# pothosware/PothosComms

Measured on NVIDIA B200. Metric: FIR Msamples/s (cf32, 256 taps) at 1/2/4/8 B200; % HBM roofline; vs host CPU, higher is better.
Workload: dtype f32

## Files before the change

### pothoscomms_b200/csrc/fir_os.cu

```cuda
#include <algorithm>
#include <cmath>
#include <complex>
#include <cstdlib>
#include <vector>

#include "bulk.cuh"
#include "fft.hpp"
#include "os64_core.cuh"

namespace b200c {

struct FirOs64Args {
    const void *in;
    void *out;
    const void *hf;
    const void *twa;
    const void *twb;
    const void *twf;
    long long n_in;
    long long n_out;
    long long in_stride, out_stride;
    int nchan;
    int K;
    int parts;
};

template <bool CONJ, bool SLOT_REV>
__device__ __forceinline__ void step_twiddle(c2 (&v)[64], const c2 *__restrict__ twa, const c2 *__restrict__ twb, const int t)
{
    c2 A[8], B[8];
#pragma unroll
    for (int i = 1; i < 8; i++) { A[i] = twa[i * 64 + t]; B[i] = twb[i * 64 + t]; }
#pragma unroll
    for (int a = 0; a < 8; a++)
#pragma unroll
        for (int b = 0; b < 8; b++) {
            const int j = 8 * a + b, r = SLOT_REV ? rev64(j) : j;
            if (a) v[r] = cmul_p<CONJ>(v[r], A[a]);
            if (b) v[r] = cmul_p<CONJ>(v[r], B[b]);
        }
}

constexpr int kBulkElems = 4098;

template <int MINB>
__global__ void __launch_bounds__(64, MINB) fir_os64_kernel(const FirOs64Args a)
{
    __shared__ __align__(16) c2 F[kOs64SmemElems];
    __shared__ __align__(8) unsigned long long bar;
    const int t = threadIdx.x;
    const c2 *__restrict__ twa = static_cast<const c2 *>(a.twa);
    const c2 *__restrict__ twb = static_cast<const c2 *>(a.twb);
    const int Km1 = a.K - 1;
    const int hop = 4096 - Km1;
    const long long nblk = (a.n_out + hop - 1) / hop;
    const long long tstep = gridDim.x, dch = tstep / nblk, dblk = tstep - dch * nblk;
    long long ch = (long long)blockIdx.x / nblk, blk = (long long)blockIdx.x - ch * nblk;
    auto bulk_src = [&](long long ch, long long blk, const c2 *&src) {
        if (ch >= a.nchan) return false;
        const long long base = blk * hop;
        const c2 *in = static_cast<const c2 *>(a.in) + ch * a.in_stride;
        const int mis = (int)(((reinterpret_cast<unsigned long long>(in) >> 3) + base) & 1);
        src = in + (base - mis);
        return base - mis >= 0 && base - mis + kBulkElems <= a.n_in;
    };
    if (t == 0) mbar_init(&bar, 1);
    __syncthreads();
    const c2 *src = nullptr;
    bool pending = bulk_src(ch, blk, src);
    if (pending && t == 0) bulk_load(F, src, kBulkElems * (unsigned)sizeof(c2), &bar);
    unsigned parity = 0;

    while (ch < a.nchan) {
        const long long base = blk * hop;
        long long nch = ch + dch, nblkpos = blk + dblk;
        if (nblkpos >= nblk) { nblkpos -= nblk; nch++; }
        const c2 *__restrict__ in = static_cast<const c2 *>(a.in) + ch * a.in_stride;
        const c2 *__restrict__ hf = static_cast<const c2 *>(a.hf) + ch * 4096;
        c2 *__restrict__ out = static_cast<c2 *>(a.out) + ch * a.out_stride;
        c2 v[64];
        if (pending) {
            const int mis = (int)(((reinterpret_cast<unsigned long long>(in) >> 3) + base) & 1);
            mbar_wait(&bar, parity);
            parity ^= 1;
#pragma unroll
            for (int n1 = 0; n1 < 64; n1++) v[rev64(n1)] = F[mis + 64 * n1 + t];
        } else {
#pragma unroll
            for (int n1 = 0; n1 < 64; n1++) {
                const long long g = base + 64 * n1 + t;
                v[rev64(n1)] = g < a.n_in ? __ldcg(in + g) : 0ull;
            }
        }
        dft64_dit<false>(v);
        step_twiddle<false, false>(v, twa, twb, t);
        __syncthreads();
#pragma unroll
        for (int k1 = 0; k1 < 64; k1++) F[k1 * kOs64Stride + t] = v[k1];
        __syncthreads();
#pragma unroll
        for (int n2 = 0; n2 < 64; n2++) v[rev64(n2)] = F[t * kOs64Stride + n2];
        dft64_dit<false>(v);
#pragma unroll
        for (int k2 = 0; k2 < 64; k2++) v[k2] = cmul_p<false>(v[k2], hf[64 * k2 + t]);
        dft64_dif<true>(v);
        step_twiddle<true, true>(v, twa, twb, t);
        __syncthreads();
#pragma unroll
        for (int n2 = 0; n2 < 64; n2++) F[t * kOs64Stride + n2] = v[rev64(n2)];
        __syncthreads();
#pragma unroll
        for (int k1 = 0; k1 < 64; k1++) v[k1] = F[k1 * kOs64Stride + t];
        __syncthreads();
        pending = bulk_src(nch, nblkpos, src);
        if (pending && t == 0) bulk_load(F, src, kBulkElems * (unsigned)sizeof(c2), &bar);
        dft64_dif<true>(v);
        c2 *o = out + (base - Km1);
        if (base + hop <= a.n_out) {
#pragma unroll
            for (int n1 = 0; n1 < 64; n1++) {
                const int i = 64 * n1 + t;
                if (i >= Km1) __stcg(o + i, v[rev64(n1)]);
            }
        } else {
#pragma unroll
            for (int n1 = 0; n1 < 64; n1++) {
                const int i = 64 * n1 + t;
                if (i >= Km1 && base + i - Km1 < a.n_out) __stcg(o + i, v[rev64(n1)]);
            }
        }
        ch = nch; blk = nblkpos;
    }
}

constexpr int kOs64Groups = 4;
__global__ void __launch_bounds__(64 * kOs64Groups, 1) fir_os64p_kernel(const FirOs64Args a)
{
    extern __shared__ __align__(16) c2 os64p_dyn[];
    __shared__ __align__(8) unsigned long long bars[kOs64Groups];
    const int g = threadIdx.x >> 6, t = threadIdx.x & 63;
    c2 *F = os64p_dyn + g * kOs64SmemElems;
    c2 *TW = os64p_dyn + kOs64Groups * kOs64SmemElems;
    c2 *HF = TW + 4096;
    unsigned long long *bar = &bars[g];
    auto gsync = [&] { asm volatile("bar.sync %0, 64;" ::"r"(g + 1) : "memory"); };
    const int Km1 = a.K - 1;
    const int hop = 4096 - Km1;
    const long long nblk = (a.n_out + hop - 1) / hop;
    const long long parts = a.parts, ntask = (long long)a.nchan * parts;
    const long long bstep = parts * kOs64Groups;
    auto bulk_src = [&](long long ch, long long blk, const c2 *&src) {
        if (ch >= a.nchan || blk >= nblk) return false;
        const long long base = blk * hop;
        const c2 *in = static_cast<const c2 *>(a.in) + ch * a.in_stride;
        const int mis = (int)(((reinterpret_cast<unsigned long long>(in) >> 3) + base) & 1);
        src = in + (base - mis);
        return base - mis >= 0 && base - mis + kBulkElems <= a.n_in;
    };
    long long task = blockIdx.x;
    if (t == 0) mbar_init(bar, 1);
    gsync();
    const c2 *src = nullptr;
    bool pending = task < ntask && bulk_src(task / parts, (task % parts) * kOs64Groups + g, src);
    if (pending && t == 0) bulk_load(F, src, kBulkElems * (unsigned)sizeof(c2), bar);
    unsigned parity = 0;
    {
        const c2 *__restrict__ twf = static_cast<const c2 *>(a.twf);
        for (int i = threadIdx.x; i < 4096; i += 64 * kOs64Groups) TW[i] = twf[i];
    }
    long long staged = -1;
    for (; task < ntask; task += gridDim.x) {
        const long long ch = task / parts, first = (task - ch * parts) * kOs64Groups + g;
        if (ch != staged) {
            const c2 *__restrict__ hfg = static_cast<const c2 *>(a.hf) + ch * 4096;
            for (int i = threadIdx.x; i < 4096; i += 64 * kOs64Groups) HF[i] = __ldg(hfg + i);
            staged = ch;
        }
        __syncthreads();
        const c2 *__restrict__ in = static_cast<const c2 *>(a.in) + ch * a.in_stride;
        c2 *__restrict__ out = static_cast<c2 *>(a.out) + ch * a.out_stride;
        for (long long blk = first; blk < nblk; blk += bstep) {
            const long long base = blk * hop;
            c2 v[64];
            if (pending) {
                const int mis = (int)(((reinterpret_cast<unsigned long long>(in) >> 3) + base) & 1);
                mbar_wait(bar, parity);
                parity ^= 1;
#pragma unroll
                for (int n1 = 0; n1 < 64; n1++) v[rev64(n1)] = F[mis + 64 * n1 + t];
            } else {
#pragma unroll
                for (int n1 = 0; n1 < 64; n1++) {
                    const long long gi = base + 64 * n1 + t;
                    v[rev64(n1)] = gi < a.n_in ? __ldcg(in + gi) : 0ull;
                }
            }
            dft64_dit<false>(v);
#pragma unroll
            for (int k1 = 1; k1 < 64; k1++) v[k1] = cmul_p<false>(v[k1], TW[k1 * 64 + t]);
            gsync();
#pragma unroll
            for (int k1 = 0; k1 < 64; k1++) F[k1 * kOs64Stride + t] = v[k1];
            gsync();
#pragma unroll
            for (int n2 = 0; n2 < 64; n2++) v[rev64(n2)] = F[t * kOs64Stride + n2];
            dft64_dit<false>(v);
#pragma unroll
            for (int k2 = 0; k2 < 64; k2++) v[k2] = cmul_p<false>(v[k2], HF[64 * k2 + t]);
            dft64_dif<true>(v);
#pragma unroll
            for (int n2 = 1; n2 < 64; n2++) v[rev64(n2)] = cmul_p<true>(v[rev64(n2)], TW[n2 * 64 + t]);
            gsync();
#pragma unroll
            for (int n2 = 0; n2 < 64; n2++) F[t * kOs64Stride + n2] = v[rev64(n2)];
            gsync();
#pragma unroll
            for (int k1 = 0; k1 < 64; k1++) v[k1] = F[k1 * kOs64Stride + t];
            gsync();
            {
                const bool last = blk + bstep >= nblk;
                const long long nt = task + gridDim.x;
                pending = last ? (nt < ntask && bulk_src(nt / parts, (nt % parts) * kOs64Groups + g, src)) : bulk_src(ch, blk + bstep, src);
                if (pending && t == 0) bulk_load(F, src, kBulkElems * (unsigned)sizeof(c2), bar);
            }
            dft64_dif<true>(v);
            c2 *o = out + (base - Km1);
            if (base + hop <= a.n_out) {
#pragma unroll
                for (int n1 = 0; n1 < 64; n1++) {
                    const int i = 64 * n1 + t;
                    if (i >= Km1) __stcg(o + i, v[rev64(n1)]);
                }
            } else {
#pragma unroll
                for (int n1 = 0; n1 < 64; n1++) {
                    const int i = 64 * n1 + t;
                    if (i >= Km1 && base + i - Km1 < a.n_out) __stcg(o + i, v[rev64(n1)]);
                }
            }
        }
        __syncthreads();
    }
}


constexpr bool kOs32PartialTwiddles = false;

template <bool CONJ, bool SLOT_REV>
__device__ __forceinline__ void twiddle32(c2 (&v)[32], const c2 *__restrict__ tw, const int t)
{
    c2 A[8], B[4];
#pragma unroll
    for (int a = 1; a < 8; a++) A[a] = tw[(4 * a) * 32 + t];
#pragma unroll
    for (int b = 1; b < 4; b++) B[b] = tw[b * 32 + t];
#pragma unroll
    for (int k = 1; k < 32; k++) {
        const int a = k >> 2, b = k & 3, r = SLOT_REV ? rev32(k) : k;
        if (a) v[r] = cmul_p<CONJ>(v[r], A[a]);
        if (b) v[r] = cmul_p<CONJ>(v[r], B[b]);
    }
}

struct FirOs32Args {
    const void *in;
    void *out;
    const void *hf;
    const void *tw;
    long long n_in, n_out;
    long long in_stride, out_stride;
    int nchan;
    int K;
    int spread;
    int pdl;
};

constexpr int kOs32Landing = 1032;
template <int WARPS, int MINB, bool TABS = false, bool PT = kOs32PartialTwiddles, bool EARLY = false>
__global__ void __launch_bounds__(32 * WARPS, MINB) fir_os32_kernel(const FirOs32Args a)
{
    extern __shared__ __align__(16) c2 os32_dyn[];
    __shared__ __align__(16) c2 Fs[TABS ? 1 : WARPS][TABS ? 1 : kOs32SmemElems];
    __shared__ __align__(8) unsigned long long bars[WARPS];
    const int t = threadIdx.x & 31, w = threadIdx.x >> 5;
    c2 *F = TABS ? os32_dyn + w * kOs32SmemElems : Fs[TABS ? 0 : w];
    unsigned long long *bar = &bars[w];
    const c2 *__restrict__ tw = static_cast<const c2 *>(a.tw);
    const c2 *__restrict__ hf_tab = nullptr;
    c2 *Lb = F;
    if constexpr (TABS && EARLY) Lb = os32_dyn + WARPS * kOs32SmemElems + 2048 + w * kOs32Landing;
    const int Km1 = a.K - 1;
    const int hop = 1024 - Km1;
    const long long nblk = (a.n_out + hop - 1) / hop;
    const long long tstep = (long long)gridDim.x * WARPS, dch = tstep / nblk, dblk = tstep - dch * nblk;
    const long long task0 = a.spread ? (long long)w * gridDim.x + blockIdx.x : (long long)blockIdx.x * WARPS + w;
    long long ch = task0 / nblk, blk = task0 - ch * nblk;
    constexpr int kBulk = 1026;
    auto bulk_src = [&](long long ch, long long blk, const c2 *&src) {
        if (ch >= a.nchan) return false;
        const long long base = blk * hop;
        const c2 *in = static_cast<const c2 *>(a.in) + ch * a.in_stride;
        const int mis = (int)(((reinterpret_cast<unsigned long long>(in) >> 3) + base) & 1);
        src = in + (base - mis);
        return base - mis >= 0 && base - mis + kBulk <= a.n_in;
    };
    if (t == 0) mbar_init(bar, 1);
    __syncwarp();
    const c2 *src = nullptr;
    bool pending = bulk_src(ch, blk, src);
    unsigned parity = 0;
    if constexpr (TABS) {
        asm volatile("griddepcontrol.launch_dependents;");
        c2 *tab = os32_dyn + WARPS * kOs32SmemElems;
        const c2 *__restrict__ hf0 = static_cast<const c2 *>(a.hf);
        if (a.pdl) {
            for (int i = threadIdx.x; i < 1024; i += 32 * WARPS) { tab[i] = hf0[i]; tab[1024 + i] = tw[i]; }
            asm volatile("griddepcontrol.wait;" ::: "memory");
            if (pending && t == 0) bulk_load(Lb, src, kBulk * (unsigned)sizeof(c2), bar);
        } else {
            if (pending && t == 0) bulk_load(Lb, src, kBulk * (unsigned)sizeof(c2), bar);
            for (int i = threadIdx.x; i < 1024; i += 32 * WARPS) { tab[i] = hf0[i]; tab[1024 + i] = tw[i]; }
        }
        __syncthreads();
        hf_tab = tab; tw = tab + 1024;
    } else {
        if (pending && t == 0) bulk_load(Lb, src, kBulk * (unsigned)sizeof(c2), bar);
    }
    while (ch < a.nchan) {
        const long long base = blk * hop;
        long long nch = ch + dch, nblkpos = blk + dblk;
        if (nblkpos >= nblk) { nblkpos -= nblk; nch++; }
        const c2 *__restrict__ in = static_cast<const c2 *>(a.in) + ch * a.in_stride;
        const c2 *__restrict__ hf = TABS ? hf_tab : static_cast<const c2 *>(a.hf) + ch * 1024;
        c2 *__restrict__ out = static_cast<c2 *>(a.out) + ch * a.out_stride;
        c2 v[32];
        if (pending) {
            const int mis = (int)(((reinterpret_cast<unsigned long long>(in) >> 3) + base) & 1);
            mbar_wait(bar, parity);
            parity ^= 1;
#pragma unroll
            for (int n1 = 0; n1 < 32; n1++) v[rev32(n1)] = Lb[mis + 32 * n1 + t];
        } else {
#pragma unroll
            for (int n1 = 0; n1 < 32; n1++) {
                const long long g = base + 32 * n1 + t;
                v[rev32(n1)] = g < a.n_in ? __ldcg(in + g) : 0ull;
            }
        }
        if constexpr (TABS && EARLY) {
            __syncwarp();
            pending = bulk_src(nch, nblkpos, src);
            if (pending && t == 0) bulk_load(Lb, src, kBulk * (unsigned)sizeof(c2), bar);
        }
        dft32_dit<false>(v);
        if constexpr (PT) twiddle32<false, false>(v, tw, t);
        else {
#pragma unroll
            for (int k1 = 1; k1 < 32; k1++) v[k1] = cmul_p<false>(v[k1], tw[k1 * 32 + t]);
        }
        __syncwarp();
#pragma unroll
        for (int k1 = 0; k1 < 32; k1++) F[k1 * kOs32Stride + t] = v[k1];
        __syncwarp();
#pragma unroll
        for (int n2 = 0; n2 < 32; n2++) v[rev32(n2)] = F[t * kOs32Stride + n2];
        dft32_dit<false>(v);
#pragma unroll
        for (int k2 = 0; k2 < 32; k2++) v[k2] = cmul_p<false>(v[k2], hf[32 * k2 + t]);
        dft32_dif<true>(v);
        if constexpr (PT) twiddle32<true, true>(v, tw, t);
        else {
#pragma unroll
            for (int n2 = 1; n2 < 32; n2++) v[rev32(n2)] = cmul_p<true>(v[rev32(n2)], tw[n2 * 32 + t]);
        }
        __syncwarp();
#pragma unroll
        for (int n2 = 0; n2 < 32; n2++) F[t * kOs32Stride + n2] = v[rev32(n2)];
        __syncwarp();
#pragma unroll
        for (int k1 = 0; k1 < 32; k1++) v[k1] = F[k1 * kOs32Stride + t];
        if constexpr (!(TABS && EARLY)) {
            __syncwarp();
            pending = bulk_src(nch, nblkpos, src);
            if (pending && t == 0) bulk_load(F, src, kBulk * (unsigned)sizeof(c2), bar);
        }
        dft32_dif<true>(v);
        c2 *o = out + (base - Km1);
        if (base + hop <= a.n_out) {
#pragma unroll
            for (int n1 = 0; n1 < 32; n1++) {
                const int i = 32 * n1 + t;
                if (i >= Km1) __stcg(o + i, v[rev32(n1)]);
            }
        } else {
#pragma unroll
            for (int n1 = 0; n1 < 32; n1++) {
                const int i = 32 * n1 + t;
                if (i >= Km1 && base + i - Km1 < a.n_out) __stcg(o + i, v[rev32(n1)]);
            }
        }
        ch = nch; blk = nblkpos;
    }
}

B200C_HD constexpr float cos48(int e)
{
    constexpr float t[48] = {
        1.0f, 0.9914448857307434f, 0.9659258127212524f, 0.9238795042037964f, 0.8660253882408142f, 0.7933533191680908f,
        0.7071067690849304f, 0.6087614297866821f, 0.5f, 0.3826834261417389f, 0.258819043636322f, 0.13052618503570557f, 0.0f,
        -0.13052618503570557f, -0.258819043636322f, -0.3826834261417389f, -0.5f, -0.6087614297866821f, -0.7071067690849304f,
        -0.7933533191680908f, -0.8660253882408142f, -0.9238795042037964f, -0.9659258127212524f, -0.9914448857307434f, -1.0f,
        -0.9914448857307434f, -0.9659258127212524f, -0.9238795042037964f, -0.8660253882408142f, -0.7933533191680908f,
        -0.7071067690849304f, -0.6087614297866821f, -0.5f, -0.3826834261417389f, -0.258819043636322f, -0.13052618503570557f, 0.0f,
        0.13052618503570557f, 0.258819043636322f, 0.3826834261417389f, 0.5f, 0.6087614297866821f, 0.7071067690849304f,
        0.7933533191680908f, 0.8660253882408142f, 0.9238795042037964f, 0.9659258127212524f, 0.9914448857307434f};
    return t[e % 48];
}
B200C_HD constexpr float sin48(int e) { return cos48(e + 36); }

B200C_HD constexpr int rev16(int k) { return 4 * (k & 3) + (k >> 2); }
template <bool INV> B200C_HD void dft16_dif(c2 (&x)[16])
{
#pragma unroll
    for (int k = 0; k < 4; k++) {
        dft4_p<INV>(x[k], x[k + 4], x[k + 8], x[k + 12]);
        x[k + 4] = mul_w64<INV>(x[k + 4], 4 * k);
        x[k + 8] = mul_w64<INV>(x[k + 8], 8 * k);
        x[k + 12] = mul_w64<INV>(x[k + 12], 12 * k);
    }
#pragma unroll
    for (int g = 0; g < 4; g++) dft4_p<INV>(x[4 * g], x[4 * g + 1], x[4 * g + 2], x[4 * g + 3]);
}

B200C_HD c2 cmul_acc(c2 f, c2 w, c2 acc)
{
    float fx, fy, wx, wy;
    upk(f, fx, fy); upk(w, wx, wy);
    return fma2(f, pk(wx, wx), fma2(pk(-fy, fx), pk(wy, wy), acc));
}

struct FirOsX32Args {
    const void *in;
    void *out;
    const void *hx;
    const void *tw;
    const void *tw3;
    long long n_in, n_out;
    long long p0;
    int m0;
    int pdl;
};
constexpr int kX32Rows = 48, kX32SmemElems = kX32Rows * kOs32Stride;

constexpr int kX32TabElems = 3072 + 1536 + 1024;
template <int WARPS, int MINB, bool PT = false, bool SPLIT = false>
__global__ void __launch_bounds__(32 * WARPS, MINB) fir_os32x_kernel(const FirOsX32Args a)
{
    extern __shared__ __align__(16) c2 x32_smem[];
    __shared__ __align__(8) unsigned long long bars[WARPS];
    const int t = threadIdx.x & 31, wp = threadIdx.x >> 5;
    const c2 *__restrict__ tw = static_cast<const c2 *>(a.tw);
    const c2 *__restrict__ tw3 = static_cast<const c2 *>(a.tw3);
    const c2 *__restrict__ hx = static_cast<const c2 *>(a.hx);
    c2 *F = x32_smem + wp * kX32SmemElems;
    c2 *const Lb = F;
    unsigned long long &bar = bars[wp];
    const c2 *__restrict__ in = static_cast<const c2 *>(a.in);
    c2 *__restrict__ out = static_cast<c2 *>(a.out);
    const int m0 = a.m0, hop_out = 1536 - m0, hop_in = hop_out / 3 * 2;
    const long long nblk = (a.n_out + hop_out - 1) / hop_out;
    constexpr int kBulk = 1026;
    auto bulk_src = [&](long long blk, const c2 *&src) {
        if (blk >= nblk) return false;
        const long long P = a.p0 + blk * hop_in;
        const int mis = (int)(((reinterpret_cast<unsigned long long>(in) >> 3) + (unsigned long long)P) & 1);
        src = in + (P - mis);
        return P - mis >= 0 && P - mis + kBulk <= a.n_in;
    };
    if (t == 0) mbar_init(&bar, 1);
    __syncwarp();
    long long blk = (long long)blockIdx.x * WARPS + wp;
    const long long bstep = (long long)gridDim.x * WARPS;
    const c2 *src = nullptr;
    bool pending = bulk_src(blk, src);
    unsigned parity = 0;
    if constexpr (WARPS > 1) {
        asm volatile("griddepcontrol.launch_dependents;");
        c2 *tab = x32_smem + WARPS * kX32SmemElems;
        auto stage = [&] {
            for (int i = threadIdx.x; i < 3072; i += 32 * WARPS) tab[i] = hx[i];
            for (int i = threadIdx.x; i < 1536; i += 32 * WARPS) tab[3072 + i] = tw3[i];
            for (int i = threadIdx.x; i < 1024; i += 32 * WARPS) tab[3072 + 1536 + i] = tw[i];
        };
        if (a.pdl) {
            stage();
            asm volatile("griddepcontrol.wait;" ::: "memory");
            if (pending && t == 0) bulk_load(Lb, src, kBulk * (unsigned)sizeof(c2), &bar);
        } else {
            if (pending && t == 0) bulk_load(Lb, src, kBulk * (unsigned)sizeof(c2), &bar);
            stage();
        }
        __syncthreads();
        hx = tab; tw3 = tab + 3072; tw = tab + 3072 + 1536;
    } else {
        if (pending && t == 0) bulk_load(Lb, src, kBulk * (unsigned)sizeof(c2), &bar);
    }
    for (; blk < nblk; blk += bstep) {
        const long long P = a.p0 + blk * hop_in;
        c2 v[32];
        if (pending) {
            const int mis = (int)(((reinterpret_cast<unsigned long long>(in) >> 3) + (unsigned long long)P) & 1);
            mbar_wait(&bar, parity);
            parity ^= 1;
#pragma unroll
            for (int n1 = 0; n1 < 32; n1++) v[rev32(n1)] = Lb[mis + 32 * n1 + t];
        } else {
#pragma unroll
            for (int n1 = 0; n1 < 32; n1++) {
                const long long g = P + 32 * n1 + t;
                v[rev32(n1)] = (g >= 0 && g < a.n_in) ? __ldcg(in + g) : 0ull;
            }
        }
        dft32_dit<false>(v);
        if constexpr (PT) twiddle32<false, false>(v, tw, t);
        else {
#pragma unroll
            for (int k1 = 1; k1 < 32; k1++) v[k1] = cmul_p<false>(v[k1], tw[k1 * 32 + t]);
        }
        __syncwarp();
#pragma unroll
        for (int k1 = 0; k1 < 32; k1++) F[k1 * kOs32Stride + t] = v[k1];
        __syncwarp();
#pragma unroll
        for (int n2 = 0; n2 < 32; n2++) v[rev32(n2)] = F[t * kOs32Stride + n2];
        dft32_dit<false>(v);
        c2 s[3][16];
#pragma unroll
        for (int c = 0; c < 16; c++) {
            const c2 xa = v[c], xb = v[c + 16];
            const c2 h0 = hx[32 * c + t], g0 = hx[1536 + 32 * c + t];
            const c2 h1 = hx[32 * (c + 16) + t], g1 = hx[1536 + 32 * (c + 16) + t];
            const c2 h2 = hx[32 * (c + 32) + t], g2 = hx[1536 + 32 * (c + 32) + t];
            s[c % 3][c / 3] = cmul_acc(xb, g0, cmul_p<false>(xa, h0));
            s[(c + 16) % 3][(c + 16) / 3] = cmul_acc(xa, g1, cmul_p<false>(xb, h1));
            s[(c + 32) % 3][(c + 32) / 3] = cmul_acc(xb, g2, cmul_p<false>(xa, h2));
        }
#pragma unroll
        for (int c1 = 0; c1 < 3; c1++) dft16_dif<true>(s[c1]);
        __syncwarp();
        c2 twb1 = 0, twb2 = 0;
        if constexpr (PT) { twb1 = tw3[16 * 32 + t]; twb2 = tw3[32 * 32 + t]; }
#pragma unroll
        for (int v2 = 0; v2 < 16; v2++) {
            const int r = rev16(v2);
// ... 758 lines not shown
static int launch_general(const FirOs32GArgs &a, long long nblk, int sm_count, cudaStream_t stream)
{
    auto kern = fir_os32g_kernel<M, MULTI_L, REAL, TILE_OUT, MINB>;
    const size_t smem = sizeof(c2) * (size_t)osg_smem_elems(a.L, TILE_OUT);
    static thread_local bool configured[16] = {false};
    int dev = 0;
    B200C_CUDA_TRY(cudaGetDevice(&dev));
    if (dev < 16 && !configured[dev]) {
        B200C_CUDA_TRY(cudaFuncSetAttribute(kern, cudaFuncAttributeMaxDynamicSharedMemorySize, 64 * 1024));
        configured[dev] = true;
    }
    const long long by_smem = std::max<long long>(1, (220 * 1024) / (long long)(smem + 1024));
    const int per_sm = (int)std::min<long long>(MINB, by_smem);
    const int grid = (int)std::min<long long>(nblk, (long long)sm_count * per_sm * 4);
    kern<<<grid, 32, smem, stream>>>(a);
    B200C_CUDA_TRY(cudaGetLastError());
    return B200C_OK;
}

template <int NW, int MINB>
static void launch_osp(const FirOs32GArgs &a, int M, size_t smem, long long nblk, int sm_count, cudaStream_t stream)
{
    auto kern = fir_osp_kernel<NW, MINB>;
    static thread_local bool configured[16] = {false};
    int dev = 0;
    if (cudaGetDevice(&dev) == cudaSuccess && dev < 16 && !configured[dev]) {
        cudaFuncSetAttribute(kern, cudaFuncAttributeMaxDynamicSharedMemorySize, 100 * 1024);
        if (const char *e = std::getenv("B200C_OSP_CARVE")) cudaFuncSetAttribute(kern, cudaFuncAttributePreferredSharedMemoryCarveout, std::atoi(e));
        configured[dev] = true;
    }
    static const int forced = [] { const char *e = std::getenv("B200C_OSP_PERSM"); return e ? std::atoi(e) : 0; }();
    const long long per_sm = std::max<long long>(1, std::min<long long>(forced > 0 ? forced : MINB, (224 * 1024) / (long long)(smem + 1024)));
    const int grid = (int)std::min<long long>(nblk, (long long)sm_count * per_sm * 2);
    kern<<<grid, 32 * NW, smem, stream>>>(a, M);
}

template <int NW, int G>
static void launch_ospg(const FirOs32GArgs &a, int M, size_t smem, long long nblk, int sm_count, cudaStream_t stream)
{
    auto kern = fir_ospg_kernel<NW, G>;
    static thread_local bool configured[16] = {false};
    int dev = 0;
    if (cudaGetDevice(&dev) == cudaSuccess && dev < 16 && !configured[dev]) {
        cudaFuncSetAttribute(kern, cudaFuncAttributeMaxDynamicSharedMemorySize, 227 * 1024);
        configured[dev] = true;
    }
    const int grid = (int)std::min<long long>((nblk + G - 1) / G, (long long)sm_count);
    kern<<<grid, 32 * NW * G, smem, stream>>>(a, M);
}

static bool pdl_enabled()
{
    static const bool on = [] { const char *e = std::getenv("B200C_PDL"); return !e || std::atoi(e) != 0; }();
    return on;
}
template <typename Kernel, typename Args>
static cudaError_t launch_dependent(Kernel kern, int grid, int block, size_t smem, cudaStream_t stream, const Args &a)
{
    cudaLaunchConfig_t cfg = {};
    cfg.gridDim = dim3((unsigned)grid); cfg.blockDim = dim3((unsigned)block); cfg.dynamicSmemBytes = smem; cfg.stream = stream;
    cudaLaunchAttribute attr[1];
    attr[0].id = cudaLaunchAttributeProgrammaticStreamSerialization;
    attr[0].val.programmaticStreamSerializationAllowed = 1;
    cfg.attrs = attr; cfg.numAttrs = 1;
    return cudaLaunchKernelEx(&cfg, kern, a);
}

int fir_os_launch(const FirOsPlan &p, const void *d_in, size_t in_elems, void *d_out, size_t nq, int sm_count,
                  cudaStream_t stream, const FirOsBatch *batch)
{
    if (nq == 0) return B200C_OK;
    const int nchan = batch ? batch->nchan : 1;
    if (p.x32) {
        if (batch) { set_error("filter bank: the batched launch serves complex float32 L = M = 1 only"); return B200C_ERR_UNSUPPORTED; }
        FirOsX32Args a;
        a.in = d_in; a.out = d_out; a.hx = p.d_hx; a.tw = p.d_tw1k; a.tw3 = p.d_tw3;
        a.n_in = (long long)in_elems; a.n_out = (long long)nq * 3; a.p0 = p.p0; a.m0 = p.m0;
        const long long nblk = (a.n_out + (1536 - p.m0) - 1) / (1536 - p.m0);
        const size_t tile = sizeof(c2) * kX32SmemElems;
        const size_t smem = 12 * tile + sizeof(c2) * kX32TabElems;
        static thread_local bool configured[16] = {false};
        int dev = 0;
        B200C_CUDA_TRY(cudaGetDevice(&dev));
        if (dev < 16 && !configured[dev]) {
            B200C_CUDA_TRY(cudaFuncSetAttribute(fir_os32x_kernel<12, 1, true, true>, cudaFuncAttributeMaxDynamicSharedMemorySize, (int)smem));
            configured[dev] = true;
        }
        const int grid = (int)std::min<long long>((nblk + 11) / 12, (long long)sm_count);
        a.pdl = pdl_enabled() ? 1 : 0;
        if (a.pdl) B200C_CUDA_TRY(launch_dependent(fir_os32x_kernel<12, 1, true, true>, grid, 32 * 12, smem, stream, a));
        else fir_os32x_kernel<12, 1, true, true><<<grid, 32 * 12, smem, stream>>>(a);
        B200C_CUDA_TRY(cudaGetLastError());
        return B200C_OK;
    }
    if (p.general) {
        if (batch) { set_error("filter bank: the batched launch serves complex float32 L = M = 1 only"); return B200C_ERR_UNSUPPORTED; }
        FirOs32GArgs a;
        a.in = d_in; a.out = d_out; a.H = p.d_H; a.tw = p.d_tw1k;
        a.n_in = (long long)in_elems; a.nq = (long long)nq; a.start0 = p.start0; a.L = p.L; a.hop = p.hopq;
        if (p.osp) {
            const int nw = std::max(p.L, p.M);
            const size_t smem = sizeof(c2) * ((size_t)p.M * kOs32SmemElems + (size_t)p.L * osp_plane_stride(p.L));
            const long long nblk = ((long long)nq + p.hopq - 1) / p.hopq;
            const size_t shared_tab = sizeof(c2) * ((size_t)p.L * p.M * 1024 + 1024);
            if (p.ospg && nw == 3) launch_ospg<3, 4>(a, p.M, shared_tab + 4 * smem, nblk, sm_count, stream);
            else if (p.ospg && nw == 2) launch_ospg<2, 6>(a, p.M, shared_tab + 6 * smem, nblk, sm_count, stream);
            else if (p.ospg && nw == 4) launch_ospg<4, 3>(a, p.M, shared_tab + 3 * smem, nblk, sm_count, stream);
            else if (nw == 2) launch_osp<2, 7>(a, p.M, smem, nblk, sm_count, stream);
            else if (nw == 3) launch_osp<3, 5>(a, p.M, smem, nblk, sm_count, stream);
            else launch_osp<4, 3>(a, p.M, smem, nblk, sm_count, stream);
            B200C_CUDA_TRY(cudaGetLastError());
            return B200C_OK;
        }
        const long long per = (long long)p.hopq * (p.real ? 2 : 1);
        const long long nblk = ((long long)nq + per - 1) / per;
        const bool ml = p.L > 1, tile = p.L >= 2 && p.L <= 4;
#define OSG(MM, RR, MB1, MBL)                                                                                      \
    (!ml ? launch_general<MM, false, RR, false, MB1>(a, nblk, sm_count, stream)                                      \
         : tile ? launch_general<MM, true, RR, true, MBL>(a, nblk, sm_count, stream)                                 \
                : launch_general<MM, true, RR, false, MBL>(a, nblk, sm_count, stream))
        if (p.M == 1) return p.real ? OSG(1, true, 12, 10) : OSG(1, false, 12, 10);
        return p.real ? OSG(2, true, 10, 8) : OSG(2, false, 10, 8);
#undef OSG
    }
    if (p.real32) {
        if (batch) { set_error("filter bank: the batched launch serves complex float32 L = M = 1 only"); return B200C_ERR_UNSUPPORTED; }
        FirOs32RArgs a;
        a.in = static_cast<const float *>(d_in); a.out = static_cast<float *>(d_out); a.hf = p.d_hf1k; a.tw = p.d_tw1k;
        a.n_in = (long long)in_elems; a.n_out = (long long)nq; a.K = p.K;
        const long long npair = ((long long)nq + p.hop() - 1) / p.hop();
        const size_t tile = sizeof(c2) * kOs32SmemElems;
        const size_t smem_early = 12 * tile + sizeof(c2) * 2048 + sizeof(c2) * 12 * kOs32Landing;
        static thread_local bool configured[16] = {false};
        int dev = 0;
        B200C_CUDA_TRY(cudaGetDevice(&dev));
        if (dev < 16 && !configured[dev]) {
            B200C_CUDA_TRY(cudaFuncSetAttribute(fir_os32r_kernel<12, 1, true>, cudaFuncAttributeMaxDynamicSharedMemorySize, (int)smem_early));
            configured[dev] = true;
        }
        const int grid = (int)std::min<long long>((npair + 11) / 12, (long long)sm_count);
        fir_os32r_kernel<12, 1, true><<<grid, 32 * 12, smem_early, stream>>>(a);
        B200C_CUDA_TRY(cudaGetLastError());
        return B200C_OK;
    }
    const size_t n_out = nq;
    const long long nblk = (((long long)n_out + p.hop() - 1) / p.hop()) * nchan;
    if (p.N == 1024) {
        FirOs32Args a;
        a.in = d_in; a.out = d_out; a.hf = batch ? batch->d_hf : p.d_hf1k; a.tw = p.d_tw1k;
        a.n_in = (long long)in_elems; a.n_out = (long long)n_out; a.K = p.K;
        a.nchan = nchan; a.in_stride = batch ? batch->in_stride : 0; a.out_stride = batch ? batch->out_stride : 0;
        a.spread = 0; a.pdl = 0;
        if (nchan == 1) {
            const size_t smem_early = sizeof(c2) * (12 * (size_t)kOs32SmemElems + 2048 + 12 * (size_t)kOs32Landing);
            static thread_local bool configured[16] = {false};
            int dev = 0;
            B200C_CUDA_TRY(cudaGetDevice(&dev));
            if (dev < 16 && !configured[dev]) {
                B200C_CUDA_TRY(cudaFuncSetAttribute(fir_os32_kernel<12, 1, true, false, true>, cudaFuncAttributeMaxDynamicSharedMemorySize, (int)smem_early));
                configured[dev] = true;
            }
            a.spread = nblk < 12LL * sm_count ? 1 : 0;
            const int grid = (int)std::min<long long>(a.spread ? nblk : (nblk + 11) / 12, (long long)sm_count);
            a.pdl = pdl_enabled() ? 1 : 0;
            if (a.pdl) B200C_CUDA_TRY(launch_dependent(fir_os32_kernel<12, 1, true, false, true>, grid, 32 * 12, smem_early, stream, a));
            else fir_os32_kernel<12, 1, true, false, true><<<grid, 32 * 12, smem_early, stream>>>(a);
            B200C_CUDA_TRY(cudaGetLastError());
            return B200C_OK;
        }
        {
            const int grid = (int)std::min<long long>(nblk, (long long)sm_count * 12 * 4);
            fir_os32_kernel<1, 12><<<grid, 32, 0, stream>>>(a);
        }
        B200C_CUDA_TRY(cudaGetLastError());
        return B200C_OK;
    }
    FirOs64Args a;
    a.in = d_in; a.out = d_out; a.hf = batch ? batch->d_hf : p.d_hf; a.twa = p.d_twa; a.twb = p.d_twb; a.twf = p.d_twf;
    a.n_in = (long long)in_elems; a.n_out = (long long)n_out; a.K = p.K;
    a.nchan = nchan; a.in_stride = batch ? batch->in_stride : 0; a.out_stride = batch ? batch->out_stride : 0;
    a.parts = 1;
    static const bool persistent = [] { const char *e = std::getenv("B200C_OS64P"); return !e || std::atoi(e) != 0; }();
    const long long blocks_per_chan = ((long long)n_out + p.hop() - 1) / p.hop();
    if (persistent && (long long)nchan * blocks_per_chan >= 4LL * kOs64Groups * sm_count) {
        const size_t smem = sizeof(c2) * ((size_t)kOs64Groups * kOs64SmemElems + 4096 + 4096);
        if (nchan == 1) a.parts = sm_count;
        else {
            const long long maxp = std::max<long long>(1, blocks_per_chan / 16);
            double best = -1.0;
            for (long long q = 1; q <= std::min<long long>(maxp, 32); q++) {
                const long long T = (long long)nchan * q, rounds = (T + sm_count - 1) / sm_count;
                const double util = (double)T / (double)(rounds * sm_count) - 1.5e-3 * (double)(q - 1);
                if (util > best) { best = util; a.parts = (int)q; }
            }
        }
        static thread_local bool configured[16] = {false};
        int dev = 0;
        B200C_CUDA_TRY(cudaGetDevice(&dev));
        if (dev < 16 && !configured[dev]) {
            B200C_CUDA_TRY(cudaFuncSetAttribute(fir_os64p_kernel, cudaFuncAttributeMaxDynamicSharedMemorySize, (int)smem));
            configured[dev] = true;
        }
        fir_os64p_kernel<<<sm_count, 64 * kOs64Groups, smem, stream>>>(a);
        B200C_CUDA_TRY(cudaGetLastError());
        return B200C_OK;
    }
    const int grid = (int)std::min<long long>(nblk, (long long)sm_count * 4 * 4);
    fir_os64_kernel<4><<<grid, 64, 0, stream>>>(a);
    B200C_CUDA_TRY(cudaGetLastError());
    return B200C_OK;
}

}
```

### pothoscomms_b200/csrc/umma.cuh

```cuda
#pragma once
#include "bulk.cuh"

namespace b200c {

__device__ __forceinline__ unsigned prmt_u(unsigned a, unsigned b, unsigned sel)
{
    unsigned r;
    asm("prmt.b32 %0, %1, %2, %3;" : "=r"(r) : "r"(a), "r"(b), "r"(sel));
    return r;
}

__device__ __forceinline__ bool elect_one()
{
    unsigned pred;
    asm volatile(
        "{\n"
        ".reg .pred p;\n"
        "elect.sync _|p, 0xffffffff;\n"
        "selp.u32 %0, 1, 0, p;\n"
        "}\n" : "=r"(pred));
    return pred != 0;
}

__device__ __forceinline__ unsigned long long umma_smem_desc(unsigned smem_addr, unsigned lbo_bytes, unsigned sbo_bytes, unsigned layout = 0)
{
    unsigned long long d = 0;
    d |= (unsigned long long)((smem_addr >> 4) & 0x3FFF);
    d |= (unsigned long long)((lbo_bytes >> 4) & 0x3FFF) << 16;
    d |= (unsigned long long)((sbo_bytes >> 4) & 0x3FFF) << 32;
    d |= 1ull << 46;
    d |= (unsigned long long)(layout & 7) << 61;
    return d;
}

__host__ __device__ constexpr unsigned umma_idesc_i8(bool a_signed, int N)
{
    return (2u << 4) | ((a_signed ? 1u : 0u) << 7) | (1u << 10) | ((unsigned)(N >> 3) << 17) | ((128u >> 4) << 24);
}

__host__ __device__ constexpr unsigned umma_idesc_i8_ab(bool a_signed, bool b_signed, int N)
{
    return (2u << 4) | ((a_signed ? 1u : 0u) << 7) | ((b_signed ? 1u : 0u) << 10) | ((unsigned)(N >> 3) << 17) | ((128u >> 4) << 24);
}

__device__ __forceinline__ void umma_i8(unsigned d_tmem, unsigned long long adesc, unsigned long long bdesc, unsigned idesc, bool accumulate)
{
    asm volatile(
        "{\n\t"
        ".reg .pred p;\n\t"
        "setp.ne.b32 p, %4, 0;\n\t"
        "tcgen05.mma.cta_group::1.kind::i8 [%0], %1, %2, %3, p;\n\t"
        "}\n" ::"r"(d_tmem), "l"(adesc), "l"(bdesc), "r"(idesc), "r"((unsigned)accumulate)
        : "memory");
}

__device__ __forceinline__ void umma_i8_first(unsigned d_tmem, unsigned long long adesc, unsigned long long bdesc, unsigned idesc)
{
    asm volatile(
        "{\n\t"
        ".reg .pred p;\n\t"
        "setp.ne.b32 p, 0, 0;\n\t"
        "tcgen05.mma.cta_group::1.kind::i8 [%0], %1, %2, %3, p;\n\t"
        "}\n" ::"r"(d_tmem), "l"(adesc), "l"(bdesc), "r"(idesc)
        : "memory");
}
__device__ __forceinline__ void umma_i8_acc(unsigned d_tmem, unsigned long long adesc, unsigned long long bdesc, unsigned idesc)
{
    asm volatile(
        "{\n\t"
        ".reg .pred p;\n\t"
        "setp.eq.b32 p, 0, 0;\n\t"
        "tcgen05.mma.cta_group::1.kind::i8 [%0], %1, %2, %3, p;\n\t"
        "}\n" ::"r"(d_tmem), "l"(adesc), "l"(bdesc), "r"(idesc)
        : "memory");
}

__device__ __forceinline__ void umma_i8_ts_first(unsigned d_tmem, unsigned a_tmem, unsigned long long bdesc, unsigned idesc)
{
    asm volatile(
        "{\n\t"
        ".reg .pred p;\n\t"
        "setp.ne.b32 p, 0, 0;\n\t"
        "tcgen05.mma.cta_group::1.kind::i8 [%0], [%1], %2, %3, p;\n\t"
        "}\n" ::"r"(d_tmem), "r"(a_tmem), "l"(bdesc), "r"(idesc)
        : "memory");
}
__device__ __forceinline__ void umma_i8_ts_acc(unsigned d_tmem, unsigned a_tmem, unsigned long long bdesc, unsigned idesc)
{
    asm volatile(
        "{\n\t"
        ".reg .pred p;\n\t"
        "setp.eq.b32 p, 0, 0;\n\t"
        "tcgen05.mma.cta_group::1.kind::i8 [%0], [%1], %2, %3, p;\n\t"
        "}\n" ::"r"(d_tmem), "r"(a_tmem), "l"(bdesc), "r"(idesc)
        : "memory");
}

__device__ __forceinline__ void tmem_ld4(unsigned taddr, unsigned (&v)[4])
{
    asm volatile("tcgen05.ld.sync.aligned.32x32b.x4.b32 {%0, %1, %2, %3}, [%4];"
                 : "=r"(v[0]), "=r"(v[1]), "=r"(v[2]), "=r"(v[3])
                 : "r"(taddr)
                 : "memory");
}

__device__ __forceinline__ void tmem_ld16(unsigned taddr, unsigned (&v)[16])
{
    asm volatile("tcgen05.ld.sync.aligned.32x32b.x16.b32 {%0, %1, %2, %3, %4, %5, %6, %7, %8, %9, %10, %11, %12, %13, %14, %15}, [%16];"
                 : "=r"(v[0]), "=r"(v[1]), "=r"(v[2]), "=r"(v[3]), "=r"(v[4]), "=r"(v[5]), "=r"(v[6]), "=r"(v[7]), "=r"(v[8]),
                   "=r"(v[9]), "=r"(v[10]), "=r"(v[11]), "=r"(v[12]), "=r"(v[13]), "=r"(v[14]), "=r"(v[15])
                 : "r"(taddr)
                 : "memory");
}

__device__ __forceinline__ void tmem_ld16x256b_x2(unsigned taddr, unsigned (&v)[8])
{
    asm volatile("tcgen05.ld.sync.aligned.16x256b.x2.b32 {%0, %1, %2, %3, %4, %5, %6, %7}, [%8];"
                 : "=r"(v[0]), "=r"(v[1]), "=r"(v[2]), "=r"(v[3]), "=r"(v[4]), "=r"(v[5]), "=r"(v[6]), "=r"(v[7])
                 : "r"(taddr)
                 : "memory");
}

__device__ __forceinline__ void mbar_arrive(unsigned long long *bar)
{
    asm volatile("mbarrier.arrive.shared::cta.b64 _, [%0];" ::"r"(smem_u32(bar)) : "memory");
}

static __device__ unsigned long long *g_umma_watch = nullptr;

__device__ __forceinline__ bool mbar_try_wait(unsigned long long *bar, unsigned parity, unsigned hint_ns = 1000000u)
{
    unsigned ok;
    asm volatile(
        "{\n"
        ".reg .pred p;\n"
        "mbarrier.try_wait.parity.shared::cta.b64 p, [%1], %2, %3;\n"
        "selp.u32 %0, 1, 0, p;\n"
        "}\n" : "=r"(ok) : "r"(smem_u32(bar)), "r"(parity), "r"(hint_ns) : "memory");
    return ok != 0;
}


__device__ __forceinline__ void timed_wait(unsigned long long *bar, unsigned parity, long long &acc)
{
    const long long t0 = clock64();
    while (!mbar_try_wait(bar, parity)) {}
    acc += clock64() - t0;
}

__device__ __forceinline__ void watched_wait(bool timed, unsigned long long *bar, unsigned parity, long long &acc)
{
    if (!timed && mbar_try_wait(bar, parity)) return;
    const long long t0 = clock64();
    bool noted = false;
    while (!mbar_try_wait(bar, parity)) {
        const long long waited = clock64() - t0;
        if (waited > (1ll << 35) && !noted) {
            noted = true;
            if (g_umma_watch) {
                g_umma_watch[blockIdx.x * 32 + (threadIdx.x >> 5)] = ((unsigned long long)smem_u32(bar) << 8) | (parity << 1) | 1ull;
                __threadfence_system();
            }
        }
        if (waited > (3ll << 34)) __trap();
    }
    acc += clock64() - t0;
}


}
```

Baseline: 301,700.

## Keep OS32 filter and twiddle tables in tensor memory instead of shared memory

In the persistent single-channel overlap-save FFT kernel, the filter spectrum and twiddle tables are staged into Blackwell tensor memory (TMEM) by warps 0-3 instead of into shared memory. The per-element multiplies then read them with tcgen05.ld instead of per-thread shared-memory loads. The aim is to cut shared-memory traffic and bank pressure and to free 16 KB of dynamic shared memory. In exchange it adds TMEM allocation and fences, plus synchronous TMEM load waits inside the hot loop. It is enabled by default through an environment variable when the non-spread path is taken.

After: 328,600 (median of 6 runs). +8.9%, better.

```diff
diff --git a/pothoscomms_b200/csrc/fir_os.cu b/pothoscomms_b200/csrc/fir_os.cu
--- a/pothoscomms_b200/csrc/fir_os.cu
+++ b/pothoscomms_b200/csrc/fir_os.cu
@@ -7,6 +7,7 @@
 #include "bulk.cuh"
 #include "fft.hpp"
 #include "os64_core.cuh"
+#include "umma.cuh"
 
 namespace b200c {
 
@@ -275,20 +276,61 @@
     int pdl;
 };
 
+constexpr unsigned kOs32TmemCols = 128;
+constexpr unsigned kOs32TmemTw = 64;
+
+__device__ __forceinline__ c2 pk_u(unsigned lo, unsigned hi) { c2 r; asm("mov.b64 %0, {%1, %2};" : "=l"(r) : "r"(lo), "r"(hi)); return r; }
+
+__device__ __forceinline__ void os32_tmem_fill(unsigned taddr, const c2 *__restrict__ hf, const c2 *__restrict__ tw, const int t)
+{
+#pragma unroll
+    for (int c = 0; c < 8; c++) {
+        const c2 *src = c < 4 ? hf + 256 * c : tw + 256 * (c - 4);
+        unsigned r[16];
+#pragma unroll
+        for (int i = 0; i < 8; i++) {
+            const c2 x = src[32 * i + t];
+            r[2 * i] = (unsigned)x;
+            r[2 * i + 1] = (unsigned)(x >> 32);
+        }
+        tmem_st16(taddr + 16 * c, r);
+    }
+    asm volatile("tcgen05.wait::st.sync.aligned;" ::: "memory");
+}
+
+template <bool CONJ, bool SLOT_REV, int J0>
+__device__ __forceinline__ void os32_tmem_mul(c2 (&v)[32], const unsigned taddr)
+{
+#pragma unroll
+    for (int c = 0; c < 2; c++) {
+        unsigned r[32];
+        tmem_ld32(taddr + 32 * c, r);
+        tmem_wait_ld32(r);
+#pragma unroll
+        for (int i = 0; i < 16; i++) {
+            const int j = 16 * c + i, s = SLOT_REV ? rev32(j) : j;
+            if (j >= J0) v[s] = cmul_p<CONJ>(v[s], pk_u(r[2 * i], r[2 * i + 1]));
+        }
+    }
+}
+
 constexpr int kOs32Landing = 1032;
-template <int WARPS, int MINB, bool TABS = false, bool PT = kOs32PartialTwiddles, bool EARLY = false>
+template <int WARPS, int MINB, bool TABS = false, bool PT = kOs32PartialTwiddles, bool EARLY = false, bool TMEM = false>
 __global__ void __launch_bounds__(32 * WARPS, MINB) fir_os32_kernel(const FirOs32Args a)
 {
+    static_assert(!TMEM || (TABS && !PT && WARPS >= 4), "the TMEM tables serve the persistent form; warps 0..3 fill them");
     extern __shared__ __align__(16) c2 os32_dyn[];
     __shared__ __align__(16) c2 Fs[TABS ? 1 : WARPS][TABS ? 1 : kOs32SmemElems];
     __shared__ __align__(8) unsigned long long bars[WARPS];
+    __shared__ unsigned tmem_base_s;
     const int t = threadIdx.x & 31, w = threadIdx.x >> 5;
     c2 *F = TABS ? os32_dyn + w * kOs32SmemElems : Fs[TABS ? 0 : w];
     unsigned long long *bar = &bars[w];
     const c2 *__restrict__ tw = static_cast<const c2 *>(a.tw);
     const c2 *__restrict__ hf_tab = nullptr;
+    unsigned tmem_lane = 0;
     c2 *Lb = F;
-    if constexpr (TABS && EARLY) Lb = os32_dyn + WARPS * kOs32SmemElems + 2048 + w * kOs32Landing;
+    if constexpr (TABS && EARLY) Lb = os32_dyn + WARPS * kOs32SmemElems + (TMEM ? 0 : 2048) + w * kOs32Landing;
     const int Km1 = a.K - 1;
     const int hop = 1024 - Km1;
     const long long nblk = (a.n_out + hop - 1) / hop;
@@ -313,16 +355,35 @@
         asm volatile("griddepcontrol.launch_dependents;");
         c2 *tab = os32_dyn + WARPS * kOs32SmemElems;
         const c2 *__restrict__ hf0 = static_cast<const c2 *>(a.hf);
+        if constexpr (TMEM) {
+            if (w == 0) {
+                asm volatile("tcgen05.alloc.cta_group::1.sync.aligned.shared::cta.b32 [%0], %1;" ::"r"(smem_u32(&tmem_base_s)), "r"(kOs32TmemCols) : "memory");
+                asm volatile("tcgen05.relinquish_alloc_permit.cta_group::1.sync.aligned;" ::: "memory");
+            }
+            asm volatile("tcgen05.fence::before_thread_sync;" ::: "memory");
+            __syncthreads();
+            asm volatile("tcgen05.fence::after_thread_sync;" ::: "memory");
+            tmem_lane = tmem_base_s + ((unsigned)(32 * (w & 3)) << 16);
+        }
+        auto stage = [&] {
+            if constexpr (TMEM) {
+                if (w < 4) os32_tmem_fill(tmem_lane, hf0, tw, t);
+            } else {
+                for (int i = threadIdx.x; i < 1024; i += 32 * WARPS) { tab[i] = hf0[i]; tab[1024 + i] = tw[i]; }
+            }
+        };
         if (a.pdl) {
-            for (int i = threadIdx.x; i < 1024; i += 32 * WARPS) { tab[i] = hf0[i]; tab[1024 + i] = tw[i]; }
+            stage();
             asm volatile("griddepcontrol.wait;" ::: "memory");
             if (pending && t == 0) bulk_load(Lb, src, kBulk * (unsigned)sizeof(c2), bar);
         } else {
             if (pending && t == 0) bulk_load(Lb, src, kBulk * (unsigned)sizeof(c2), bar);
-            for (int i = threadIdx.x; i < 1024; i += 32 * WARPS) { tab[i] = hf0[i]; tab[1024 + i] = tw[i]; }
-        }
+            stage();
+        }
+        if constexpr (TMEM) asm volatile("tcgen05.fence::before_thread_sync;" ::: "memory");
         __syncthreads();
-        hf_tab = tab; tw = tab + 1024;
+        if constexpr (TMEM) asm volatile("tcgen05.fence::after_thread_sync;" ::: "memory");
+        else { hf_tab = tab; tw = tab + 1024; }
     } else {
         if (pending && t == 0) bulk_load(Lb, src, kBulk * (unsigned)sizeof(c2), bar);
     }
@@ -353,7 +414,8 @@
             if (pending && t == 0) bulk_load(Lb, src, kBulk * (unsigned)sizeof(c2), bar);
         }
         dft32_dit<false>(v);
-        if constexpr (PT) twiddle32<false, false>(v, tw, t);
+        if constexpr (TMEM) os32_tmem_mul<false, false, 1>(v, tmem_lane + kOs32TmemTw);
+        else if constexpr (PT) twiddle32<false, false>(v, tw, t);
         else {
 #pragma unroll
             for (int k1 = 1; k1 < 32; k1++) v[k1] = cmul_p<false>(v[k1], tw[k1 * 32 + t]);
@@ -365,10 +427,14 @@
 #pragma unroll
         for (int n2 = 0; n2 < 32; n2++) v[rev32(n2)] = F[t * kOs32Stride + n2];
         dft32_dit<false>(v);
-#pragma unroll
-        for (int k2 = 0; k2 < 32; k2++) v[k2] = cmul_p<false>(v[k2], hf[32 * k2 + t]);
+        if constexpr (TMEM) os32_tmem_mul<false, false, 0>(v, tmem_lane);
+        else {
+#pragma unroll
+            for (int k2 = 0; k2 < 32; k2++) v[k2] = cmul_p<false>(v[k2], hf[32 * k2 + t]);
+        }
         dft32_dif<true>(v);
-        if constexpr (PT) twiddle32<true, true>(v, tw, t);
+        if constexpr (TMEM) os32_tmem_mul<true, true, 1>(v, tmem_lane + kOs32TmemTw);
+        else if constexpr (PT) twiddle32<true, true>(v, tw, t);
         else {
 #pragma unroll
             for (int n2 = 1; n2 < 32; n2++) v[rev32(n2)] = cmul_p<true>(v[rev32(n2)], tw[n2 * 32 + t]);
@@ -400,6 +466,12 @@
             }
         }
         ch = nch; blk = nblkpos;
+    }
+    if constexpr (TMEM) {
+        asm volatile("tcgen05.fence::before_thread_sync;" ::: "memory");
+        __syncthreads();
+        asm volatile("tcgen05.fence::after_thread_sync;" ::: "memory");
+        if (w == 0) asm volatile("tcgen05.dealloc.cta_group::1.sync.aligned.b32 %0, %1;" ::"r"(tmem_base_s), "r"(kOs32TmemCols) : "memory");
     }
 }
 
@@ -1464,19 +1536,21 @@
         a.nchan = nchan; a.in_stride = batch ? batch->in_stride : 0; a.out_stride = batch ? batch->out_stride : 0;
         a.spread = 0; a.pdl = 0;
         if (nchan == 1) {
-            const size_t smem_early = sizeof(c2) * (12 * (size_t)kOs32SmemElems + 2048 + 12 * (size_t)kOs32Landing);
-            static thread_local bool configured[16] = {false};
+            a.spread = nblk < 12LL * sm_count ? 1 : 0;
+            const bool tmem = !a.spread && [] { const char *e = std::getenv("B200C_OS32_TMEM"); return !e || std::atoi(e) != 0; }();
+            const auto kern = tmem ? fir_os32_kernel<12, 1, true, false, true, true> : fir_os32_kernel<12, 1, true, false, true>;
+            const size_t smem_early = sizeof(c2) * (12 * (size_t)kOs32SmemElems + (tmem ? 0 : 2048) + 12 * (size_t)kOs32Landing);
+            static thread_local bool configured[2][16] = {};
             int dev = 0;
             B200C_CUDA_TRY(cudaGetDevice(&dev));
-            if (dev < 16 && !configured[dev]) {
-                B200C_CUDA_TRY(cudaFuncSetAttribute(fir_os32_kernel<12, 1, true, false, true>, cudaFuncAttributeMaxDynamicSharedMemorySize, (int)smem_early));
-                configured[dev] = true;
-            }
-            a.spread = nblk < 12LL * sm_count ? 1 : 0;
+            if (dev < 16 && !configured[tmem][dev]) {
+                B200C_CUDA_TRY(cudaFuncSetAttribute(kern, cudaFuncAttributeMaxDynamicSharedMemorySize, (int)smem_early));
+                configured[tmem][dev] = true;
+            }
             const int grid = (int)std::min<long long>(a.spread ? nblk : (nblk + 11) / 12, (long long)sm_count);
             a.pdl = pdl_enabled() ? 1 : 0;
-            if (a.pdl) B200C_CUDA_TRY(launch_dependent(fir_os32_kernel<12, 1, true, false, true>, grid, 32 * 12, smem_early, stream, a));
-            else fir_os32_kernel<12, 1, true, false, true><<<grid, 32 * 12, smem_early, stream>>>(a);
+            if (a.pdl) B200C_CUDA_TRY(launch_dependent(kern, grid, 32 * 12, smem_early, stream, a));
+            else kern<<<grid, 32 * 12, smem_early, stream>>>(a);
             B200C_CUDA_TRY(cudaGetLastError());
             return B200C_OK;
         }
diff --git a/pothoscomms_b200/csrc/umma.cuh b/pothoscomms_b200/csrc/umma.cuh
--- a/pothoscomms_b200/csrc/umma.cuh
+++ b/pothoscomms_b200/csrc/umma.cuh
@@ -110,6 +110,35 @@
                  : "=r"(v[0]), "=r"(v[1]), "=r"(v[2]), "=r"(v[3]), "=r"(v[4]), "=r"(v[5]), "=r"(v[6]), "=r"(v[7]), "=r"(v[8]),
                    "=r"(v[9]), "=r"(v[10]), "=r"(v[11]), "=r"(v[12]), "=r"(v[13]), "=r"(v[14]), "=r"(v[15])
                  : "r"(taddr)
+                 : "memory");
+}
+
+__device__ __forceinline__ void tmem_ld32(unsigned taddr, unsigned (&v)[32])
+{
+    asm volatile("tcgen05.ld.sync.aligned.32x32b.x32.b32 {%0, %1, %2, %3, %4, %5, %6, %7, %8, %9, %10, %11, %12, %13, %14, %15, %16, %17, %18, %19, %20, %21, %22, %23, %24, %25, %26, %27, %28, %29, %30, %31}, [%32];"
+                 : "=r"(v[0]), "=r"(v[1]), "=r"(v[2]), "=r"(v[3]), "=r"(v[4]), "=r"(v[5]), "=r"(v[6]), "=r"(v[7]), "=r"(v[8]),
+                   "=r"(v[9]), "=r"(v[10]), "=r"(v[11]), "=r"(v[12]), "=r"(v[13]), "=r"(v[14]), "=r"(v[15]),
+                   "=r"(v[16]), "=r"(v[17]), "=r"(v[18]), "=r"(v[19]), "=r"(v[20]), "=r"(v[21]), "=r"(v[22]), "=r"(v[23]), "=r"(v[24]),
+                   "=r"(v[25]), "=r"(v[26]), "=r"(v[27]), "=r"(v[28]), "=r"(v[29]), "=r"(v[30]), "=r"(v[31])
+                 : "r"(taddr)
+                 : "memory");
+}
+__device__ __forceinline__ void tmem_wait_ld32(unsigned (&v)[32])
+{
+    asm volatile("tcgen05.wait::ld.sync.aligned;"
+                 : "+r"(v[0]), "+r"(v[1]), "+r"(v[2]), "+r"(v[3]), "+r"(v[4]), "+r"(v[5]), "+r"(v[6]), "+r"(v[7]), "+r"(v[8]),
+                   "+r"(v[9]), "+r"(v[10]), "+r"(v[11]), "+r"(v[12]), "+r"(v[13]), "+r"(v[14]), "+r"(v[15]),
+                   "+r"(v[16]), "+r"(v[17]), "+r"(v[18]), "+r"(v[19]), "+r"(v[20]), "+r"(v[21]), "+r"(v[22]), "+r"(v[23]), "+r"(v[24]),
+                   "+r"(v[25]), "+r"(v[26]), "+r"(v[27]), "+r"(v[28]), "+r"(v[29]), "+r"(v[30]), "+r"(v[31])
+                 :
+                 : "memory");
+}
+
+__device__ __forceinline__ void tmem_st16(unsigned taddr, const unsigned (&v)[16])
+{
+    asm volatile("tcgen05.st.sync.aligned.32x32b.x16.b32 [%0], {%1, %2, %3, %4, %5, %6, %7, %8, %9, %10, %11, %12, %13, %14, %15, %16};"
+                 ::"r"(taddr), "r"(v[0]), "r"(v[1]), "r"(v[2]), "r"(v[3]), "r"(v[4]), "r"(v[5]), "r"(v[6]), "r"(v[7]), "r"(v[8]),
+                   "r"(v[9]), "r"(v[10]), "r"(v[11]), "r"(v[12]), "r"(v[13]), "r"(v[14]), "r"(v[15])
                  : "memory");
 }
 
```
